# sundy-li/databend

Hardware: AMD Instinct MI355X
Metric: input rows/sec aggregated (filter + hash GROUP BY), % HBM roofline (higher is better)
Workload: dtype int16 key / u64 count; 1 GPU; clickbench_q8_adv_engine_id; rows_per_gpu=100000000, input_copies=4, groups=32, selected_rows=629660, parallelism=single

## Files before the change

databend_amd/csrc/abi_exp.hpp:

```cpp
#pragma once
#include "abi_internal.hpp"

static int exp_fused_fin(dbg_agg_handle* h, const FinState& F, FusedFin& ff) {
    const Spec& S = h->spec;
    {
        static const bool dense_on = X_ENV("DBG_X_DENSE") && X_ENV("DBG_X_DENSE")[0] == '1';
        const int kt = S.key_types[0].type;
        const u32 kw = (kt == DBG_INT8 || kt == DBG_UINT8) ? 1 : ((kt == DBG_INT16 || kt == DBG_UINT16) ? 2 : 0);
        const bool co = S.n_aggs == 1 && S.aggs[0].kind == DBG_AGG_COUNT && S.aggs[0].arg_type < 0 && S.aggs[0].w0 == 1;
        if (dense_on && kw && co && h->def_clean && S.n_keys == 1) {
            if (!h->dense) {
                RETURN_IF(h->dense.ensure(65536 + 1024));
                HIPCHECK(hipMemsetAsync(h->dense, 0, (65536 + 1024) * 8, h->stream));
            }
            ff.dense = h->dense;
            ff.dense_n = kw == 1 ? 256u : 65536u;
        }
    }
    static u64* x_trace = nullptr;
    static std::vector<u64> x_init;
    if (kPhaseTrace && X_ENV("DBG_X_TRACE")) {
        if (!x_trace) {
            RETURN_IF(dev_alloc((void**)&x_trace, 4096 * 128));
            x_init.assign(16, 0);
            x_init[0] = x_init[1] = ~0ULL;
            atexit([] {
                std::vector<u64> hb(4096 * 16);
                hipDeviceSynchronize();
                hipMemcpy(hb.data(), x_trace, hb.size() * 8, hipMemcpyDeviceToHost);
                std::vector<std::vector<double>> d(14);
                for (int k = 0; k < 4096; ++k) {
                    const u64* r = &hb[k * 16];
                    if (r[0] == 0 || r[0] == ~0ULL || r[6] == 0) continue;
                    for (int p = 1; p <= 14; ++p) d[p - 1].push_back((double)(r[p] - r[0]) * 0.01);
                }
                const char* nm[] = {"first WG stream end", "last WG stream end", "last block_flush end",
                                    "ticket (last WG)", "table copied", "finalize end", "fin: scanned",
                                    "fin: groups written", "fin: bits packed", "fin: counters read",
                                    "tail: view+counts", "tail: prefix", "tail: t0 loads", "tail: t0 merged"};
                for (int p = 0; p < 14; ++p) {
                    if (d[p].empty()) continue;
                    std::sort(d[p].begin(), d[p].end());
                    fprintf(stderr, "trace %-22s median %7.2f us  (n=%zu)\n", nm[p], d[p][d[p].size() / 2], d[p].size());
                }
            });
        }
        ff.trace = x_trace + (F.seq & 4095) * 16;
        HIPCHECK(hipMemcpyAsync(ff.trace, x_init.data(), 128, hipMemcpyHostToDevice, h->stream));
    }
    return DBG_OK;
}

static int exp_pp_trace(dbg_agg_handle* h, PPAggOut& o) {
    static u64* x_pptrace = nullptr;
    if (kPhaseTrace && X_ENV("DBG_X_PPTRACE")) {
        if (!x_pptrace) {
            RETURN_IF(dev_alloc((void**)&x_pptrace, 64));
            HIPCHECK(hipMemset(x_pptrace, 0, 64));
            atexit([] {
                u64 v[8];
                hipDeviceSynchronize();
                hipMemcpy(v, x_pptrace, 64, hipMemcpyDeviceToHost);
                const double n = v[5] ? (double)v[5] : 1.0;
                fprintf(stderr, "pptrace raw us/partition [0..4] %.2f %.2f %.2f %.2f %.2f (spec kernel: load+hash, stage, insert, "
                                "emit, barriers)\n", v[0] * 0.01 / n, v[1] * 0.01 / n, v[2] * 0.01 / n, v[3] * 0.01 / n, v[4] * 0.01 / n);
                fprintf(stderr, "pptrace partitions %llu groups/partition %.0f  per partition us: insert %.2f sync %.2f "
                                "atomic %.2f write %.2f tail %.2f\n", (unsigned long long)v[5], v[6] / n, v[0] * 0.01 / n,
                        v[1] * 0.01 / n, v[2] * 0.01 / n, v[3] * 0.01 / n, v[4] * 0.01 / n);
            });
        }
        o.trace = x_pptrace;
// ... 4 lines not shown
```

databend_amd/csrc/abi_finalize.hip:

```cpp
#include "abi_exp.hpp"

static void note_observed(dbg_agg_handle* h) {
    const u64 rows = h->table_rows > h->remerged ? h->table_rows - h->remerged : 0;
    if (h->pp || !rows) return;
    h->obs_rows = rows;
    h->obs_groups = h->n_groups;
}

static void publish_groups(const dbg_agg_handle* h, uint64_t* n_groups, uint64_t* string_bytes) {
    if (n_groups) *n_groups = h->n_groups;
    if (string_bytes)
        for (int c = 0; c < h->spec.n_keys; ++c) string_bytes[c] = h->string_bytes[c];
}

bool groups_known(dbg_agg_handle* h, u64 groups, const u64* str_tot, const FinState* caps, uint64_t* n_groups,
                  uint64_t* string_bytes) {
    const Spec& S = h->spec;
    h->n_groups = groups;
    note_observed(h);
    h->string_bytes.assign(S.n_keys, 0);
    bool short_buf = caps && groups > caps->max_groups;
    for (int c = 0; c < S.n_keys; ++c) {
        if (S.key_types[c].type != DBG_STRING) continue;
        h->string_bytes[c] = str_tot[c];
// ... 252 lines not shown
        if (e != hipSuccess) return fail(DBG_ERR_DEVICE, std::string("partitioned insert (direct stage): ") + hipGetErrorString(e));
        launch_finish_outputs(h->stream, od, totals, S.n_keys, S.n_aggs);
    } else if (fuse) {
        FusedFin ff;
        ff.out = od;
        ff.totals = totals;
        ff.host_mirror = h->hcounters_dev;
        ff.seq = F.seq;
        ff.recycle = h->recycle;
        ff.on = 1;
        ff.table_empty = h->def_clean ? 1 : 0;
        ff.chain_tagged = 0;
        ff.trace = nullptr;
        ff.dense = nullptr;
        ff.dense_n = 0;
        if ((F.seq / FIN_SEQ_TAG_PERIOD) != h->scr_period) {
            HIPCHECK(hipMemsetAsync(h->scratch, 0, scr_words(h->scr_blocks, (u32)S.stride_words) * 8, h->stream));
            h->scr_period = F.seq / FIN_SEQ_TAG_PERIOD;
        }
        RETURN_IF(exp_fused_fin(h, F, ff));
        h->def_on = false;
        prof::Scope ps("agg_insert", h->stream);
        note_insert(h, launch_insert(h->stream, h->dspec, S, h->dbatches, h->def_bid, h->def_rows, false, t, true, &h->def_hb, &ff));
    } else if (small) {
        prof::Scope ps("finalize_small", h->stream);
        launch_finalize_small(h->stream, h->dspec, h->dbatches, t, od, totals, F.zero_copy ? h->hcounters_dev : nullptr,
                              h->recycle && F.zero_copy, F.seq);
    } else {
        prof::Scope ps("write_results", h->stream);
        launch_write_results(h->stream, h->dspec, S, h->dbatches, t, h->d_pos, h->d_str_pos, od);
        launch_finish_outputs(h->stream, od, totals, S.n_keys, S.n_aggs);
    }
    if (!F.zero_copy) {
        HIPCHECK(hipMemcpyAsync(h->hcounters, h->counters, CNT_WORDS * 8, hipMemcpyDeviceToHost, h->stream));
        HIPCHECK(hipMemcpyAsync(h->hcounters + CNT_WORDS, totals, 8 * (S.n_keys + 1), hipMemcpyDeviceToHost, h->stream));
    }
    F.active = true;
    return DBG_OK;
}

static int fin_complete(dbg_agg_handle* h, bool* retry, uint64_t* n_groups, uint64_t* string_bytes) {
    FinState& F = h->fin;
    *retry = false;
    F.active = false;
    if (h->pp) return pp_fin_complete(h, n_groups, string_bytes);
    bool recycled = false;
// ... 3 lines not shown
    } else {
        volatile u64* hseq = h->hcounters + CNT_WORDS + 2 + DBG_MAX_KEYS;
        volatile u64* hcomp = h->hcounters + MIRROR_COMPACT;
        bool seen = false, compact = false;
        auto t0 = std::chrono::steady_clock::now();
        for (u64 it = 0;; ++it) {
            if (__atomic_load_n(hseq, __ATOMIC_ACQUIRE) == F.seq) {
                seen = true;
                break;
            }
            const u64 cw = __atomic_load_n(hcomp, __ATOMIC_ACQUIRE);
            if ((cw >> 25) == (F.seq & ((1ULL << 39) - 1))) {
                for (int w = 0; w < CNT_WORDS; ++w) h->hcounters[w] = 0;
                h->hcounters[CNT_CLAIMS] = cw & 0xFFFFFF;
                h->hcounters[CNT_WORDS] = cw & 0xFFFFFF;
                for (int c = 0; c < DBG_MAX_KEYS; ++c) h->hcounters[CNT_WORDS + 1 + c] = 0;
                h->hcounters[CNT_WORDS + 1 + DBG_MAX_KEYS] = (cw >> 24) & 1;
                seen = compact = true;
                break;
            }
            if ((it & 255) == 255 && std::chrono::steady_clock::now() - t0 > std::chrono::milliseconds(20)) break;
            __builtin_ia32_pause();
        }
        if (!seen) HIPCHECK(hipStreamSynchronize(h->stream));
        HIPCHECK(hipGetLastError());
        recycled = h->hcounters[CNT_WORDS + 1 + DBG_MAX_KEYS] != 0;
    }
    h->uploads_pending = false;
    if (F.direct) {
        F.direct = false;
        if (h->hcounters[CNT_WORDS] == ~0ULL) {
            h->def_part = true;
            RETURN_IF(part_flush(h));
            *retry = true;
            return DBG_OK;
        }
        h->hcounters[CNT_CLAIMS] = h->hcounters[CNT_WORDS];
        recycled = true;
    }
    RETURN_IF(err_bits_fail(h->hcounters[CNT_ERR], ERR_OVF_LOST | ERR_MINMAX_SPIN | ERR_CHAIN_SPIN | ERR_FIXED_INCOMPLETE));
    if (h->hcounters[CNT_OVF_ROWS] || h->hcounters[CNT_OVF_RECS]) {
        RETURN_IF(resolve_overflow(h));
        *retry = true;
        return DBG_OK;
    }
    h->pending_rows = h->pending_recs = 0;
    const u64* tot = h->hcounters + CNT_WORDS;
// ... 98 lines not shown
    for (int a = 0; a < h->spec.n_aggs; ++a)
        if (h->src_kinds[a] == DBG_AGG_AVG_SQL)
            return fail(DBG_ERR_UNSUPPORTED, "serialized states: SQL avg is sum and count in the reference plan");
    return result_impl(h, out_states, out_keys, on_device, true);
}

int dbg_agg_finalize_into(dbg_agg_handle* h, dbg_out_column* out_aggs, dbg_out_column* out_keys, uint64_t max_groups,
                          const uint64_t* max_string_bytes, uint64_t* n_groups, uint64_t* string_bytes) {
    RETURN_IF(dbg_agg_finalize_into_async(h, out_aggs, out_keys, max_groups, max_string_bytes));
    return dbg_agg_finalize_wait(h, n_groups, string_bytes);
}

int dbg_agg_finalize_into_async(dbg_agg_handle* h, dbg_out_column* out_aggs, dbg_out_column* out_keys, uint64_t max_groups,
                                const uint64_t* max_string_bytes) {
    if (!h || !out_aggs || !out_keys) return fail(DBG_ERR_INVALID, "null argument");
    if (has_str_minmax(h->spec))
        return fail(DBG_ERR_UNSUPPORTED, std::string("dbg_agg_finalize_into_async: ") + handle_local_reason(h->spec));
    if (h->fin.active) return fail(DBG_ERR_INVALID, "a finalize is already in flight: dbg_agg_finalize_wait first");
    HIPCHECK(hipSetDevice(h->device));
    RETURN_IF(fin_setup(h, out_aggs, out_keys, max_groups, max_string_bytes));
    return fin_launch(h);
}

int dbg_agg_finalize_wait(dbg_agg_handle* h, uint64_t* n_groups, uint64_t* string_bytes) {
    if (!h || !n_groups) return fail(DBG_ERR_INVALID, "null argument");
    if (!h->fin.active) return fail(DBG_ERR_INVALID, "no finalize in flight");
    HIPCHECK(hipSetDevice(h->device));
    RETURN_IF(flush_pending(h));
    for (int round = 0; round < 3; ++round) {
        if (round) RETURN_IF(fin_launch(h));
        bool retry = false;
        int rc = fin_complete(h, &retry, n_groups, string_bytes);
        if (rc != DBG_OK || !retry) return rc;
    }
    return fail(DBG_ERR_INTERNAL, "finalize did not converge");
}
}
```

databend_amd/csrc/agg.hip:

```cpp
#include <cstdlib>
#include <cstring>
#include <limits>
#include <type_traits>

#include "legacy.hpp"
#include "agg.hpp"
#include <hip/hip_ext.h>
#include "agg_dev.hpp"

#define BLOCK 256
#define SLOTS_PER_THREAD 8
#define SLOTS_PER_BLOCK (BLOCK * SLOTS_PER_THREAD)
#define LDS_BUDGET_BYTES (32 * 1024)
#define LDS_PROBE_CAP 64
#define FLUSH_ROUND 16



__device__ __forceinline__ u64 pack_key(const Spec& S, const DCol* keys, u64 i) {
    u64 k = 0;
    for (int c = 0; c < S.n_keys; ++c) {
        const DCol& col = keys[c];
        bool v = dcol_valid(col, i);
        if (col.nullable) k |= (u64)(v ? 1 : 0) << (8 * S.voff[c]);
// ... 2430 lines not shown
        default: return v >= k;
    }
}

template <typename T>
__device__ __forceinline__ T vget(const v4u& y, int j) {
    constexpr int W = sizeof(T);
    if constexpr (W == 8) {
        u32 lo = j ? y.z : y.x, hi = j ? y.w : y.y;
        return (T)(((u64)hi << 32) | lo);
    } else {
        int wi = (j * W) >> 2;
        u32 word = wi == 0 ? y.x : (wi == 1 ? y.y : (wi == 2 ? y.z : y.w));
        return (T)(word >> (((j * W) & 3) * 8));
    }
}

#define WQ 128
#define WQW 384

template <typename T, bool PRED, int NT, bool CO>
__global__ void __launch_bounds__(NT) agg_insert_fast_kernel(const Spec* __restrict__ spec, const BatchDesc* __restrict__ batches,
                                                               u32 bid, u64 rows, TableDesc t, u32 lds_slots,
                                                               T lo, T hi, int negate, FusedFin ff) {
    extern __shared__ __attribute__((aligned(16))) u64 lds[];
    constexpr int V = 16 / sizeof(T);
    const Spec& S = *spec;
    const BatchDesc& B = batches[bid];
    const T* __restrict__ col = (const T*)B.keys[0].data;
    const u32 sw = S.stride_words;
    u32* lcount = (u32*)(lds + (u64)lds_slots * sw);
    const u32 lmask = lds_slots - 1;
    const u32 llimit = lds_slots - lds_slots / 4;
    const int lane = threadIdx.x & 63, wave = threadIdx.x >> 6;
    u64* qkey = lds + (u64)lds_slots * sw + 2 + (u64)wave * WQW;
    u64* qrow = qkey + WQ;
    v4u* vq = (v4u*)qkey;
    u64* vqb = qkey + 2 * WQ;
    if (kPhaseTrace && ff.trace && threadIdx.x == 0) atomicMin((unsigned long long*)ff.trace, (unsigned long long)__builtin_amdgcn_s_memrealtime());
    lds_table_init<false>(S, lds, lds_slots, sw, NT);
    if (threadIdx.x < 4) lcount[threadIdx.x] = 0;
    __syncthreads();
    u32 my_claims = 0;
    u32 my_ovf = 0;

    auto pass = [&](T v) -> bool { return ((v >= lo) & (v <= hi)) ^ (negate != 0); };

    auto process = [&](u64 key, u64 i) {
        int ls = lds_find<true>(S, batches, nullptr, i, key, 0, lds, lmask, sw, lcount, llimit);
        if (ls >= 0) {
            wptr<AS_LDS> st = asp<AS_LDS>(lds + (u64)ls * sw);
            if (CO) at_add<AS_LDS>(st + 1, 1ULL);
            else apply_row<AS_LDS, false, false>(S, st, B, i, batches, bid);
            return;
        }
        bool claimed;
        u64 gs = g_find<true>(S, batches, nullptr, i, key, 0, t, t.probe_limit, claimed);
        if (gs == ~0ULL) {
            push_ovf_row(t, bid, i);
            my_ovf++;
            return;
        }
        my_claims += claimed ? 1 : 0;
        wptr<AS_GLB> gst = asp<AS_GLB>(t.slots + gs * t.stride_words);
        if (CO) at_add<AS_GLB>(gst + 1, 1ULL);
// ... 135 lines not shown
                    qkey[pos] = key_of(y[u], j);
                    qrow[pos] = base[u] + j;
                    pos++;
                }
            }
            qn += tot;
            while (qn >= 64) {
                __builtin_amdgcn_wave_barrier();
                drain64();
            }
        } else {
#pragma unroll
            for (int u = 0; u < FAST_UNROLL; ++u) {
                u32 mm = m[u];
                while (mm) {
                    int j = __builtin_ctz(mm);
                    mm &= mm - 1;
                    process(key_of(y[u], j), base[u] + j);
                }
            }
        }
    };

    const u64 nvec = rows / V;
    gv4p vp = (gv4p)col;
    const u64 gstride = (u64)gridDim.x * NT;
    u64 k = (u64)blockIdx.x * NT + threadIdx.x;
    const u64 step = (u64)FAST_UNROLL * gstride;
    const u64 lastv = nvec ? nvec - 1 : 0;
    constexpr u64 TAIL_CH = (u64)NT * FAST_UNROLL;
    const bool dyn = TAIL_ON && ff.on && t.scratch != nullptr && gridDim.x > 1 && gridDim.x <= t.scr_blocks;
    u64 nstat = nvec, nch = 0;
    if (dyn) {
        nstat = ((nvec * 4 / 5) / step) * step;
        nch = (nvec - nstat + TAIL_CH - 1) / TAIL_CH;
    }
    u64 tail_grab = 0;
    if (dyn && nch && threadIdx.x == 0) tail_grab = atomicAdd((unsigned long long*)(t.counters + CNT_TAIL), 1ULL);
    v4u y[FAST_UNROLL];
#pragma unroll
    for (int u = 0; u < FAST_UNROLL; ++u) {
        u64 idx = k + u * gstride;
        y[u] = __builtin_nontemporal_load(vp + (idx < nstat ? idx : lastv));
    }
    while (__ballot(k < nstat) != 0) {
        const u64 kn = k + step;
        v4u yn[FAST_UNROLL];
#pragma unroll
        for (int u = 0; u < FAST_UNROLL; ++u) {
            u64 idx = kn + u * gstride;
            yn[u] = __builtin_nontemporal_load(vp + (idx < nstat ? idx : lastv));
        }
        u64 bases[FAST_UNROLL];
        u32 actm = 0;
#pragma unroll
        for (int u = 0; u < FAST_UNROLL; ++u) {
            u64 idx = k + u * gstride;
            actm |= (idx < nstat ? 1u : 0u) << u;
            bases[u] = idx * V;
        }
        handle_group(y, bases, FAST_UNROLL, actm);
#pragma unroll
        for (int u = 0; u < FAST_UNROLL; ++u) y[u] = yn[u];
        k = kn;
    }
    if (dyn && nch) {
        __shared__ u32 tail_id[2];
// ... 67 lines not shown
    }
    if (ff.on && t.scratch != nullptr && gridDim.x > 1 && gridDim.x <= t.scr_blocks) {
        if constexpr (CO && sizeof(T) <= 2) {
            if (kChainTagged && ff.chain_tagged && lds_slots <= 4 * NT) {
                fused_chain_tagged<T>(S, batches, B, lds, lds_slots, sw, lcount, NT, t, my_claims, my_ovf, ff);
                return;
            }
        }
        fused_chain<T, CO>(S, batches, B, lds, lds_slots, sw, lcount, NT, t, my_claims, my_ovf, ff);
        return;
    }
    block_flush<true, false, false, false>(S, batches, B, lds, lds_slots, sw, lcount, NT, t, my_claims);
    if (kPhaseTrace && ff.trace && threadIdx.x == 0) atomicMax((unsigned long long*)ff.trace + 3, (unsigned long long)__builtin_amdgcn_s_memrealtime());
    if (ff.on) fused_finalize(S, batches, t, lds, ff);
}


bool prof_ext_events(hipEvent_t* a, hipEvent_t* b);

static size_t fast_shmem(size_t table_bytes) { return table_bytes + (size_t)(1024 / 64) * WQW * 8; }
static size_t fast_table_bytes(const Spec& S) { return (size_t)lds_slots_for(S, 16 * 1024) * S.stride_words * 8 + 16; }

template <typename T>
static void launch_fast_t(hipStream_t s, const Spec* dspec, const BatchDesc* batches, u32 bid, u64 rows, const TableDesc& t,
                          u32 lslots, size_t table_bytes, bool pred, int op, i64 c, int count_only, const FusedFin* fused) {
    constexpr u64 V = 16 / sizeof(T);
    typedef __int128 W;
    const W tmin = (W)std::numeric_limits<T>::min(), tmax = (W)std::numeric_limits<T>::max();
    const W C = std::is_signed<T>::value ? (W)c : (W)(u64)c;
    W lo = 1, hi = 0;
    int neg = 0;
    auto all = [&]() { lo = tmin; hi = tmax; };
    switch (op) {
        case DBG_CMP_EQ: if (C >= tmin && C <= tmax) lo = hi = C; break;
        case DBG_CMP_NE: neg = 1; if (C >= tmin && C <= tmax) lo = hi = C; break;
        case DBG_CMP_LT: if (C > tmax) all(); else if (C > tmin) { lo = tmin; hi = C - 1; } break;
        case DBG_CMP_LE: if (C >= tmax) all(); else if (C >= tmin) { lo = tmin; hi = C; } break;
        case DBG_CMP_GT: if (C < tmin) all(); else if (C < tmax) { lo = C + 1; hi = tmax; } break;
        default: if (C <= tmin) all(); else if (C <= tmax) { lo = C; hi = tmax; } break;
    }
    if (lo > hi) { lo = 1; hi = 0; }
    const int nt = 1024;
    static_assert(FIN_NT == 1024, "the fused finalize runs on the insert's workgroup");
    static const u64 x_grid = X_ENV("DBG_X_FAST_GRID") ? (u64)atoll(X_ENV("DBG_X_FAST_GRID")) : 0;
    const u64 max_blocks = (x_grid && fused && fused->dense) ? x_grid : 256;
    size_t shmem = fast_shmem(table_bytes);
    FusedFin ff;
    if (fused) ff = *fused;
    else memset(&ff, 0, sizeof(ff));
    u64 quantum = V * (u64)nt * FAST_UNROLL;
    u64 blocks = (rows + quantum - 1) / quantum;
    if (blocks > max_blocks) blocks = max_blocks;
    if (blocks > DBG_INSERT_MAX_BLOCKS) blocks = DBG_INSERT_MAX_BLOCKS;
    if (blocks < 1) blocks = 1;
    static_assert(FAST_UNROLL >= 1 && V * 1024 * FAST_UNROLL < (1ULL << CNT1_BITS), "one grid round of a workgroup fits a level-1 count");
    ff.chain_tagged = blocks <= CHAIN_TAGGED_MAX_BLOCKS && rows / blocks + V * (u64)nt + V < (1ULL << CNT1_BITS);
    hipEvent_t ev0 = nullptr, ev1 = nullptr;
    const bool ext = prof_ext_events(&ev0, &ev1);
#define FAST_LAUNCH(P, N, F)                                                                                                     \
    do {                                                                                                                         \
        if (ext)                                                                                                                 \
            hipExtLaunchKernelGGL((agg_insert_fast_kernel<T, P, N, F>), dim3((u32)blocks), dim3(N), shmem, s, ev0, ev1, 0, dspec, \
                                  batches, bid, rows, t, lslots, (T)lo, (T)hi, neg, ff);                                        \
        else                                                                                                                     \
            hipLaunchKernelGGL((agg_insert_fast_kernel<T, P, N, F>), dim3((u32)blocks), dim3(N), shmem, s, dspec, batches, bid, \
                               rows, t, lslots, (T)lo, (T)hi, neg, ff);                                                          \
    } while (0)
    if (count_only) {
        if (pred) FAST_LAUNCH(true, 1024, true); else FAST_LAUNCH(false, 1024, true);
    } else {
        if (pred) FAST_LAUNCH(true, 1024, false); else FAST_LAUNCH(false, 1024, false);
    }
#undef FAST_LAUNCH
}

static bool fast_eligible(const Spec& S, const BatchDesc& hb, bool records) {
    if (records || !S.inline_keys || S.n_keys != 1 || S.key_types[0].nullable) return false;
    for (int a = 0; a < S.n_aggs; ++a)
        if ((S.aggs[a].kind == DBG_AGG_MIN || S.aggs[a].kind == DBG_AGG_MAX) && S.aggs[a].mmk == MMK_STR) return false;
    for (int a = 0; a < S.n_aggs; ++a)
        if (S.aggs[a].arg_type == DBG_DECIMAL256) return false;
    const DCol& k = hb.keys[0];
    int ty = k.type;
    bool intlike = (ty >= DBG_INT8 && ty <= DBG_UINT64) || ty == DBG_DATE || ty == DBG_TIMESTAMP;
    if (!intlike || k.layout != LAYOUT_ARROW || ((uintptr_t)k.data & 15)) return false;
    if (hb.n_nodes == 0) return true;
    if (hb.n_nodes != 1) return false;
    const DNode& n = hb.nodes[0];
    const DCol& f = hb.fcols[n.col];
    return n.op == DBG_PRED_CMP_CONST && f.data == k.data && f.type == ty && !f.nullable;
}

bool insert_can_fuse(const Spec& S, const BatchDesc& hb, u64 cap) {
    return hb.rows > 0 && fast_eligible(S, hb, false) && cap + 1 <= FUSED_FIN_SLOTS &&
           (cap + 1) * S.stride_words * 8 <= fast_shmem(fast_table_bytes(S));
}

InsertPath launch_insert(hipStream_t s, const Spec* dspec, const Spec& S, const BatchDesc* batches, u32 bid, u64 rows, bool records,
                         const TableDesc& t, bool use_lds, const BatchDesc* hb, const FusedFin* fused) {
    if (rows == 0) return INS_NONE;
    if (hb && use_lds && fast_eligible(S, *hb, records)) {
        u32 lslots = lds_slots_for(S, 16 * 1024);
        size_t shmem = fast_table_bytes(S);
        bool pred = hb->n_nodes == 1;
        int op = pred ? hb->nodes[0].cmp : 0;
        i64 c = pred ? hb->nodes[0].i64v : 0;
        int count_only = S.n_aggs == 1 && S.aggs[0].kind == DBG_AGG_COUNT && S.aggs[0].arg_type < 0 && S.aggs[0].w0 == 1;
        const InsertPath path = pred ? INS_FAST_PRED : INS_FAST;
        switch (hb->keys[0].type) {
            case DBG_INT8: launch_fast_t<int8_t>(s, dspec, batches, bid, rows, t, lslots, shmem, pred, op, c, count_only, fused); return path;
            case DBG_UINT8: launch_fast_t<uint8_t>(s, dspec, batches, bid, rows, t, lslots, shmem, pred, op, c, count_only, fused); return path;
            case DBG_INT16: launch_fast_t<int16_t>(s, dspec, batches, bid, rows, t, lslots, shmem, pred, op, c, count_only, fused); return path;
            case DBG_UINT16: launch_fast_t<uint16_t>(s, dspec, batches, bid, rows, t, lslots, shmem, pred, op, c, count_only, fused); return path;
            case DBG_INT32: case DBG_DATE: launch_fast_t<int32_t>(s, dspec, batches, bid, rows, t, lslots, shmem, pred, op, c, count_only, fused); return path;
            case DBG_UINT32: launch_fast_t<uint32_t>(s, dspec, batches, bid, rows, t, lslots, shmem, pred, op, c, count_only, fused); return path;
            case DBG_INT64: case DBG_TIMESTAMP: launch_fast_t<int64_t>(s, dspec, batches, bid, rows, t, lslots, shmem, pred, op, c, count_only, fused); return path;
            case DBG_UINT64: launch_fast_t<uint64_t>(s, dspec, batches, bid, rows, t, lslots, shmem, pred, op, c, count_only, fused); return path;
        }
    }
    if (!records && use_lds && hb && S.kc_word && t.cap + 1 > SHORT_MAX_SLOTS && str1_eligible(S, *hb, rows)) {
        const u32 lsw = (u32)S.kc_word + 1 + KC_KEY_WORDS;
        static const u32 x_mode = X_ENV("DBG_X_STR1") ? (u32)atoi(X_ENV("DBG_X_STR1")) : 0;
        static const u32 x_lds = X_ENV("DBG_X_STR1_LDS") ? (u32)atoi(X_ENV("DBG_X_STR1_LDS")) * 1024 : STR1_LDS_BUDGET;
        static const u32 fper = X_ENV("DBG_X_STR1_FLUSH") ? (u32)atoi(X_ENV("DBG_X_STR1_FLUSH")) : 4;
        u32 ls = 1;
        while ((ls * 2) * lsw * 8 <= x_lds) ls *= 2;
        const size_t shmem = (size_t)ls * lsw * 8 + 32 + (size_t)STR1_QCAP * 8;
        u64 blocks = (rows + (u64)STR1_NT * 16 - 1) / ((u64)STR1_NT * 16);
        if (blocks > DBG_INSERT_MAX_BLOCKS) blocks = DBG_INSERT_MAX_BLOCKS;
        if (blocks < 1) blocks = 1;
        u64 rpb = ((rows + blocks - 1) / blocks + 1) & ~1ULL;
        blocks = (rows + rpb - 1) / rpb;
        if (hb->n_nodes) hipLaunchKernelGGL(agg_insert_str1_kernel<true>, dim3((u32)blocks), dim3(STR1_NT), shmem, s, dspec, batches, bid, rows, rpb, t, ls, fper, x_mode);
        else hipLaunchKernelGGL(agg_insert_str1_kernel<false>, dim3((u32)blocks), dim3(STR1_NT), shmem, s, dspec, batches, bid, rows, rpb, t, ls, fper, x_mode);
        return hb->n_nodes ? INS_STR1_PRED : INS_STR1;
    }
    u32 lslots = use_lds ? lds_slots_for(S, LDS_BUDGET_BYTES) : 1;
    static const int x_short = X_ENV("DBG_X_SHORT") ? atoi(X_ENV("DBG_X_SHORT")) : 1;
    static const u32 x_rep = X_ENV("DBG_X_SHORT_REP") ? (u32)atoi(X_ENV("DBG_X_SHORT_REP")) : 0;
    const bool x_noshort = x_short == 0;
// ... 402 lines not shown
```

databend_amd/ffi.py:

```python
from __future__ import annotations

import ctypes as C
import os

from . import abi

_HERE = os.path.dirname(os.path.abspath(__file__))
LIB_PATH = os.environ.get("DBGPU_LIB") or os.path.join(_HERE, "libdbgpu_agg.so")
_LIB = None

EXPORTED = [
    "dbg_version", "dbg_last_error", "dbg_device_count", "dbg_agg_result_type", "dbg_agg_create",
    "dbg_agg_destroy", "dbg_agg_set_stream", "dbg_agg_reset", "dbg_agg_add_groups", "dbg_agg_finalize",
    "dbg_agg_result", "dbg_agg_finalize_into", "dbg_agg_set_recycle", "dbg_agg_set_partition_keys", "dbg_agg_finalize_into_async", "dbg_agg_finalize_wait", "dbg_agg_record_width", "dbg_agg_partition", "dbg_agg_export_records",
    "dbg_agg_merge_records", "dbg_agg_export_fixed", "dbg_agg_capacity", "dbg_agg_merge_fixed", "dbg_filter_select", "dbg_take_fixed", "dbg_sort_limit_indices", "dbg_sort_limit_multi", "dbg_agg_compact", "dbg_agg_retained_bytes", "dbg_prof_enable", "dbg_prof_reset",
    "dbg_prof_get", "dbg_prof_marker", "dbg_datagen", "dbg_agg_set_strategy", "dbg_agg_get_strategy", "dbg_agg_get_pp_stats", "dbg_agg_insert_paths",
    "dbg_agg_record_layout", "dbg_agg_set_host_staging", "dbg_agg_result_string_bytes",
    "dbg_take_string", "dbg_legacy_hash_method", "dbg_legacy_group_hash", "dbg_agg_serialized_stride", "dbg_agg_result_serialized", "dbg_agg_merge_serialized", "dbg_comm_get_unique_id", "dbg_comm_create", "dbg_comm_destroy", "dbg_agg_exchange",
    "dbg_agg_payload_counts", "dbg_agg_payload_export", "dbg_agg_payload_import", "dbg_agg_exchange_payload",
    "dbg_payload_exchange_plan", "dbg_merge_exchange_plan", "dbg_agg_payload_counts_from", "dbg_agg_payload_export_from",
    "dbg_agg_payload_import_chunks", "dbg_agg_exchange_payload_chunk",
    "dbg_scan_create", "dbg_scan_destroy", "dbg_parquet_chunk_rows", "dbg_parquet_decode",
    "dbg_native_decode", "dbg_like_pattern_kind", "dbg_like_match_host", "dbg_like_kernel_counts", "dbg_like_force_kernel",
]


class DbgError(RuntimeError):

    def __init__(self, code: int, msg: str):
        super().__init__(f"[{code}] {msg}")
        self.code = code


class DecimalOverflow(DbgError):
    pass


# ... 22 lines not shown
        L.dbg_agg_destroy.restype = None
        L.dbg_agg_set_stream.argtypes = [VP, VP]
        L.dbg_agg_reset.argtypes = [VP]
        L.dbg_agg_add_groups.argtypes = [VP, P(abi.dbg_column), P(abi.dbg_column), P(abi.dbg_filter), U64, C.c_int]
        L.dbg_agg_finalize.argtypes = [VP, P(U64), P(U64)]
        L.dbg_agg_result.argtypes = [VP, P(abi.dbg_out_column), P(abi.dbg_out_column), C.c_int]
        L.dbg_agg_result_string_bytes.argtypes = [VP, P(U64)]
        L.dbg_agg_finalize_into.argtypes = [VP, P(abi.dbg_out_column), P(abi.dbg_out_column), U64, P(U64), P(U64), P(U64)]
        L.dbg_agg_set_recycle.argtypes = [VP, C.c_int]
        L.dbg_agg_set_partition_keys.argtypes = [VP, C.c_int]
        L.dbg_agg_set_host_staging.argtypes = [VP, U64]
        L.dbg_comm_get_unique_id.argtypes = [VP]
        L.dbg_comm_create.argtypes = [VP, C.c_int, C.c_int, C.c_int, P(VP)]
        L.dbg_comm_destroy.argtypes = [VP]
        L.dbg_comm_destroy.restype = None
        L.dbg_agg_exchange.argtypes = [VP, VP, VP, P(abi.dbg_exchange_stats)]
        L.dbg_agg_set_strategy.argtypes = [VP, C.c_int]
        L.dbg_agg_record_layout.argtypes = [P(abi.dbg_agg_params), P(abi.dbg_record_layout)]
        L.dbg_agg_get_strategy.argtypes = [VP, P(C.c_int), P(U64)]
        L.dbg_agg_get_pp_stats.argtypes = [VP, P(C.c_uint32), P(U64)]
        L.dbg_agg_insert_paths.argtypes = [VP, P(U64), I32]
        L.dbg_agg_finalize_into_async.argtypes = [VP, P(abi.dbg_out_column), P(abi.dbg_out_column), U64, P(U64)]
        L.dbg_agg_finalize_wait.argtypes = [VP, P(U64), P(U64)]
        L.dbg_agg_record_width.argtypes = [VP, P(C.c_uint32)]
        L.dbg_agg_partition.argtypes = [VP, C.c_uint32, C.c_int, P(U64), P(U64)]
        L.dbg_agg_export_records.argtypes = [VP, VP, VP]
        L.dbg_agg_merge_records.argtypes = [VP, VP, VP, I32, P(U64), P(U64)]
        L.dbg_agg_export_fixed.argtypes = [VP, VP, U64]
        L.dbg_agg_capacity.argtypes = [VP, P(U64)]
        L.dbg_agg_merge_fixed.argtypes = [VP, VP, I32, U64]
        L.dbg_filter_select.argtypes = [P(abi.dbg_filter), U64, VP, P(U64), VP]
        L.dbg_take_fixed.argtypes = [P(abi.dbg_column), VP, U64, VP, VP, VP]
        L.dbg_agg_serialized_stride.argtypes = [VP, P(C.c_uint32)]
        L.dbg_agg_result_serialized.argtypes = [VP, P(abi.dbg_out_column), P(abi.dbg_out_column), C.c_int]
        L.dbg_agg_merge_serialized.argtypes = [VP, P(abi.dbg_column), P(abi.dbg_column), U64, C.c_int]
        L.dbg_legacy_hash_method.argtypes = [P(abi.dbg_datatype), C.c_int, P(C.c_int), P(C.c_uint32)]
        L.dbg_legacy_group_hash.argtypes = [P(abi.dbg_column), C.c_int, U64, VP, VP, C.c_int, VP]
        L.dbg_take_string.argtypes = [P(abi.dbg_column), VP, U64, VP, VP, U64, VP, P(U64), VP]
        L.dbg_sort_limit_indices.argtypes = [P(abi.dbg_column), U64, C.c_int, C.c_int, U64, VP, P(U64), VP]
        L.dbg_agg_compact.argtypes = [VP, P(C.c_int)]
        L.dbg_agg_retained_bytes.argtypes = [VP, P(U64)]
        L.dbg_sort_limit_multi.argtypes = [P(abi.dbg_column), C.c_int, P(C.c_int), P(C.c_int), U64, U64, VP, P(U64), VP]
        L.dbg_prof_enable.argtypes = [C.c_int]
        L.dbg_prof_get.argtypes = [C.c_int, P(C.c_char_p), P(C.c_double), P(U64)]
        L.dbg_prof_marker.argtypes = [VP]
        L.dbg_agg_payload_counts.argtypes = [VP, P(U64), P(C.c_uint32)]
# ... 57 lines not shown
```

databend_amd/workloads.py:

```python
from __future__ import annotations

import ctypes as C
import math
import time
from dataclasses import dataclass
from typing import Dict, List, Optional

import numpy as np

from . import abi
from . import column as col
from .aggregates import AggregateFunctionFactory
from .aggregator import AggregateHashTable, AggregatorParams, HashTableConfig
from .column import Column, DataType
from .device import DeviceColumn, empty
from .ffi import check, lib
from .filter import FilterProgram, cmp

BASE_SEED = 0xDA7ABE7D
F = AggregateFunctionFactory.instance()


def _torch():
    import torch
# ... 224 lines not shown
            break
        return self._publish(o, n.value, list(sb))

    def finalize_async(self, h, parity=0):
        o = self._outset(parity)
        check(lib().dbg_agg_finalize_into_async(h, o.oa, o.ok, o.cap, o.scap))

    def finalize_wait(self, h, parity=0):
        n = C.c_uint64()
        sb = (C.c_uint64 * len(self.shape.keys))()
        o = self._outset(parity)
        rc = lib().dbg_agg_finalize_wait(h, C.byref(n), sb)
        if rc == abi.DBG_ERR_INVALID and (n.value > o.cap or any(x > y for x, y in zip(sb, o.scap))):
            self._alloc_out(int(n.value * 1.25) + 1, [int(x * 1.25) + 1 for x in sb], parity)
            return self.finalize_into(h, parity)
        check(rc)
        return self._publish(o, n.value, list(sb))

    def enable_pipeline(self, mode: str = ""):
        import os
        torch = _torch()
        if getattr(self, "tables", None):
            return
        self.pipe_mode = mode or os.environ.get("DBG_PIPE_MODE", "single")
        t1 = AggregateHashTable(self.params, HashTableConfig(True, self._capacity_hint))
        check(lib().dbg_agg_set_recycle(t1.h, 1))
        self.tables = [self.table, t1]
        sa = torch.cuda.Stream()
        self.streams = [sa, sa if self.pipe_mode == "single" else torch.cuda.Stream()]
        for t, st in zip(self.tables, self.streams):
            t.set_stream(st)
        self._inflight = None

    def pipe_step(self, k: int):
        p = k % 2
        t = self.tables[p]
        self.insert(k, t)
        self.finalize_async(t.h, p)
        n = self.pipe_drain()
        self._inflight = (t.h, p)
        return n

    def pipe_drain(self):
        f, self._inflight = getattr(self, "_inflight", None), None
        return self.finalize_wait(*f) if f else 0

    def results_host(self):
        keys = [c.to_host_n(self.n_groups) if hasattr(c, "to_host_n") else _dev_to_host(c, self.n_groups) for c in self.out_keys]
        aggs = [_dev_to_host(c, self.n_groups) for c in self.out_aggs]
        return keys, aggs

    def close(self):
        for t in getattr(self, "tables", None) or [self.table]:
            t.close()


class _OutSet:

    def __init__(self, runner, cap, scap):
        self.aggs = [empty(t, cap) for t in runner.result_types]
        self.keys = [empty(t, cap, string_bytes=scap[j]) for j, t in enumerate(runner.params.group_data_types)]
# ... 47 lines not shown
```

include/dbgpu_agg.h:

```cpp
#ifndef DBGPU_AGG_H
#define DBGPU_AGG_H

#include <stdint.h>

#ifdef __cplusplus
extern "C" {
#endif

#define DBG_ABI_VERSION 1

enum {
    DBG_OK = 0,
    DBG_ERR_OVERFLOW = 1,
    DBG_ERR_OOM = 2,
    DBG_ERR_UNSUPPORTED = 3,
    DBG_ERR_INTERNAL = 4,
    DBG_ERR_INVALID = 5,
    DBG_ERR_DEVICE = 6
};

typedef enum {
    DBG_INT8 = 0,
    DBG_INT16 = 1,
    DBG_INT32 = 2,
// ... 122 lines not shown
int dbg_agg_set_stream(dbg_agg_handle* h, void* hip_stream);
int dbg_agg_reset(dbg_agg_handle* h);

int dbg_agg_add_groups(dbg_agg_handle* h, const dbg_column* group_cols, const dbg_column* arg_cols,
                       const dbg_filter* filter, uint64_t rows, int on_device);

int dbg_agg_finalize(dbg_agg_handle* h, uint64_t* n_groups, uint64_t* string_bytes);

int dbg_agg_result(dbg_agg_handle* h, dbg_out_column* out_aggs, dbg_out_column* out_keys, int on_device);
int dbg_agg_result_string_bytes(dbg_agg_handle* h, uint64_t* agg_string_bytes );
int dbg_agg_serialized_stride(dbg_agg_handle* h, uint32_t* stride );
int dbg_agg_result_serialized(dbg_agg_handle* h, dbg_out_column* out_states, dbg_out_column* out_keys, int on_device);

int dbg_agg_merge_serialized(dbg_agg_handle* h, const dbg_column* state_cols, const dbg_column* group_cols, uint64_t rows,
                             int on_device);

int dbg_agg_finalize_into(dbg_agg_handle* h, dbg_out_column* out_aggs, dbg_out_column* out_keys,
                          uint64_t max_groups, const uint64_t* max_string_bytes, uint64_t* n_groups,
                          uint64_t* string_bytes);

int dbg_agg_finalize_into_async(dbg_agg_handle* h, dbg_out_column* out_aggs, dbg_out_column* out_keys,
                                uint64_t max_groups, const uint64_t* max_string_bytes);
int dbg_agg_finalize_wait(dbg_agg_handle* h, uint64_t* n_groups, uint64_t* string_bytes);

int dbg_agg_set_recycle(dbg_agg_handle* h, int on);
int dbg_agg_set_partition_keys(dbg_agg_handle* h, int n_keys);

int dbg_agg_set_host_staging(dbg_agg_handle* h, uint64_t rows);

enum { DBG_STRATEGY_AUTO = 0, DBG_STRATEGY_TABLE = 1, DBG_STRATEGY_PARTITIONED = 2 };
int dbg_agg_set_strategy(dbg_agg_handle* h, int strategy);
int dbg_agg_get_strategy(dbg_agg_handle* h, int* partitioned, uint64_t* extra_rounds);
int dbg_agg_get_pp_stats(dbg_agg_handle* h, uint32_t* final_bits, uint64_t* spilled_partitions);
enum {
    DBG_INSERT_GENERIC = 0,
    DBG_INSERT_GENERIC_LENPRED = 1,
    DBG_INSERT_FAST = 2,
    DBG_INSERT_FAST_PRED = 3,
    DBG_INSERT_STR1 = 4,
    DBG_INSERT_STR1_PRED = 5,
    DBG_INSERT_SHORT = 6,
    DBG_INSERT_PP_GENERIC = 7,
    DBG_INSERT_PP_FIXED = 8,
    DBG_INSERT_PP_STR = 9,
    DBG_INSERT_N_PATHS = 10
};
// ... 94 lines not shown
```

Baseline: 2533 billion rows/s.

## Add single-call step API, dual-stream pipeline default, and early key-column prefetch

Adds dbg_agg_step_async, which does reset, add_groups, finalize setup and launch in one FFI call, and routes the Python pipeline through it to cut per-step host overhead. The default pipeline mode changes from a single shared stream to 'dual', which uses the default (None) streams. The fast insert kernel now takes the key pointer and stride as kernel arguments instead of loading them from device descriptors, and issues the first unrolled nontemporal loads before the LDS table init, replacing __syncthreads with a raw waitcnt plus barrier. Trace instrumentation is also restructured to measure the host gap between launches; the stream-mode change alters ordering semantics and may add overlap or contention.

```diff
diff --git a/databend_amd/csrc/abi_exp.hpp b/databend_amd/csrc/abi_exp.hpp
--- a/databend_amd/csrc/abi_exp.hpp
+++ b/databend_amd/csrc/abi_exp.hpp
@@ -1,5 +1,74 @@
 #pragma once
 #include "abi_internal.hpp"
+
+struct XTrace {
+    u64* ring = nullptr;
+    u64 launches = 0;
+    std::vector<u64> init;
+    std::chrono::steady_clock::time_point seen_at;
+    bool seen = false;
+    std::vector<double> host_us;
+};
+inline XTrace& x_tr() {
+    static XTrace x;
+    return x;
+}
+inline bool x_trace_on() {
+    static const bool on = kPhaseTrace && X_ENV("DBG_X_TRACE");
+    return on;
+}
+inline void exp_completion_seen() {
+    if (!x_trace_on()) return;
+    x_tr().seen_at = std::chrono::steady_clock::now();
+    x_tr().seen = true;
+}
+inline void exp_launch_returned() {
+    XTrace& X = x_tr();
+    if (!x_trace_on() || !X.seen) return;
+    X.host_us.push_back(std::chrono::duration<double, std::micro>(std::chrono::steady_clock::now() - X.seen_at).count());
+    X.seen = false;
+}
+inline void x_trace_dump() {
+    XTrace& X = x_tr();
+    std::vector<u64> hb(4096 * 16);
+    hipDeviceSynchronize();
+    hipMemcpy(hb.data(), X.ring, hb.size() * 8, hipMemcpyDeviceToHost);
+    auto median_line = [](const char* what, std::vector<double>& v) {
+        if (v.empty()) return;
+        std::sort(v.begin(), v.end());
+        fprintf(stderr, "trace %-44s median %7.2f us  min %7.2f  max %7.2f  (n=%zu)\n", what, v[v.size() / 2], v.front(), v.back(),
+                v.size());
+    };
+    auto whole = [](const u64* r) { return r[0] != 0 && r[0] != ~0ULL && r[1] != ~0ULL && r[6] != 0; };
+    std::vector<std::vector<double>> d(14);
+    for (int k = 0; k < 4096; ++k) {
+        const u64* r = &hb[k * 16];
+        if (!whole(r)) continue;
+        for (int p = 1; p <= 14; ++p)
+            if (r[p]) d[p - 1].push_back((double)(r[p] - r[0]) * 0.01);
+    }
+    const char* nm[] = {"first WG stream end", "last WG stream end", "last block_flush end",
+                        "ticket (last WG)", "table copied", "finalize end", "fin: scanned",
+                        "fin: groups written", "fin: bits packed", "fin: counters read",
+                        "tail: view+counts", "tail: prefix", "tail: t0 loads", "tail: t0 merged"};
+    for (int p = 0; p < 14; ++p) {
+        if (d[p].empty()) continue;
+        std::sort(d[p].begin(), d[p].end());
+        fprintf(stderr, "trace %-22s median %7.2f us  (n=%zu)\n", nm[p], d[p][d[p].size() / 2], d[p].size());
+    }
+    std::vector<double> vs_stream, vs_fin;
+    const u64 n = X.launches, first = n > 4096 ? n - 4096 : 0;
+    for (u64 j = first; j + 1 < n; ++j) {
+        const u64* a = &hb[(j & 4095) * 16];
+        const u64* b = &hb[((j + 1) & 4095) * 16];
+        if (!whole(a) || !whole(b)) continue;
+        vs_stream.push_back((double)(int64_t)(b[0] - a[1]) * 0.01);
+        vs_fin.push_back((double)(int64_t)(b[0] - a[6]) * 0.01);
+    }
+    median_line("next first WG start - first WG stream end", vs_stream);
+    median_line("next first WG start - finalize end", vs_fin);
+    median_line("host: completion seen -> next launch returned", X.host_us);
+}
 
 static int exp_fused_fin(dbg_agg_handle* h, const FinState& F, FusedFin& ff) {
     const Spec& S = h->spec;
@@ -17,36 +86,16 @@
             ff.dense_n = kw == 1 ? 256u : 65536u;
         }
     }
-    static u64* x_trace = nullptr;
-    static std::vector<u64> x_init;
-    if (kPhaseTrace && X_ENV("DBG_X_TRACE")) {
-        if (!x_trace) {
-            RETURN_IF(dev_alloc((void**)&x_trace, 4096 * 128));
-            x_init.assign(16, 0);
-            x_init[0] = x_init[1] = ~0ULL;
-            atexit([] {
-                std::vector<u64> hb(4096 * 16);
-                hipDeviceSynchronize();
-                hipMemcpy(hb.data(), x_trace, hb.size() * 8, hipMemcpyDeviceToHost);
-                std::vector<std::vector<double>> d(14);
-                for (int k = 0; k < 4096; ++k) {
-                    const u64* r = &hb[k * 16];
-                    if (r[0] == 0 || r[0] == ~0ULL || r[6] == 0) continue;
-                    for (int p = 1; p <= 14; ++p) d[p - 1].push_back((double)(r[p] - r[0]) * 0.01);
-                }
-                const char* nm[] = {"first WG stream end", "last WG stream end", "last block_flush end",
-                                    "ticket (last WG)", "table copied", "finalize end", "fin: scanned",
-                                    "fin: groups written", "fin: bits packed", "fin: counters read",
-                                    "tail: view+counts", "tail: prefix", "tail: t0 loads", "tail: t0 merged"};
-                for (int p = 0; p < 14; ++p) {
-                    if (d[p].empty()) continue;
-                    std::sort(d[p].begin(), d[p].end());
-                    fprintf(stderr, "trace %-22s median %7.2f us  (n=%zu)\n", nm[p], d[p][d[p].size() / 2], d[p].size());
-                }
-            });
+    if (x_trace_on()) {
+        XTrace& X = x_tr();
+        if (!X.ring) {
+            RETURN_IF(dev_alloc((void**)&X.ring, 4096 * 128));
+            X.init.assign(16, 0);
+            X.init[0] = X.init[1] = ~0ULL;
+            atexit(x_trace_dump);
         }
-        ff.trace = x_trace + (F.seq & 4095) * 16;
-        HIPCHECK(hipMemcpyAsync(ff.trace, x_init.data(), 128, hipMemcpyHostToDevice, h->stream));
+        ff.trace = X.ring + (X.launches++ & 4095) * 16;
+        HIPCHECK(hipMemcpyAsync(ff.trace, X.init.data(), 128, hipMemcpyHostToDevice, h->stream));
     }
     return DBG_OK;
 }
diff --git a/databend_amd/csrc/abi_finalize.hip b/databend_amd/csrc/abi_finalize.hip
--- a/databend_amd/csrc/abi_finalize.hip
+++ b/databend_amd/csrc/abi_finalize.hip
@@ -298,6 +298,7 @@
         h->def_on = false;
         prof::Scope ps("agg_insert", h->stream);
         note_insert(h, launch_insert(h->stream, h->dspec, S, h->dbatches, h->def_bid, h->def_rows, false, t, true, &h->def_hb, &ff));
+        exp_launch_returned();
     } else if (small) {
         prof::Scope ps("finalize_small", h->stream);
         launch_finalize_small(h->stream, h->dspec, h->dbatches, t, od, totals, F.zero_copy ? h->hcounters_dev : nullptr,
@@ -347,7 +348,8 @@
             if ((it & 255) == 255 && std::chrono::steady_clock::now() - t0 > std::chrono::milliseconds(20)) break;
             __builtin_ia32_pause();
         }
-        if (!seen) HIPCHECK(hipStreamSynchronize(h->stream));
+        if (seen) exp_completion_seen();
+        else HIPCHECK(hipStreamSynchronize(h->stream));
         HIPCHECK(hipGetLastError());
         recycled = h->hcounters[CNT_WORDS + 1 + DBG_MAX_KEYS] != 0;
     }
@@ -492,6 +494,19 @@
     return fin_launch(h);
 }
 
+int dbg_agg_step_async(dbg_agg_handle* h, const dbg_column* group_cols, const dbg_column* arg_cols, const dbg_filter* filter,
+                       uint64_t rows, dbg_out_column* out_aggs, dbg_out_column* out_keys, uint64_t max_groups,
+                       const uint64_t* max_string_bytes) {
+    if (!h || !group_cols || !out_aggs || !out_keys) return fail(DBG_ERR_INVALID, "null argument");
+    if (has_str_minmax(h->spec))
+        return fail(DBG_ERR_UNSUPPORTED, std::string("dbg_agg_step_async: ") + handle_local_reason(h->spec));
+    if (h->fin.active) return fail(DBG_ERR_INVALID, "a finalize is already in flight: dbg_agg_finalize_wait first");
+    RETURN_IF(dbg_agg_reset(h));
+    RETURN_IF(dbg_agg_add_groups(h, group_cols, arg_cols, filter, rows, 1));
+    RETURN_IF(fin_setup(h, out_aggs, out_keys, max_groups, max_string_bytes));
+    return fin_launch(h);
+}
+
 int dbg_agg_finalize_wait(dbg_agg_handle* h, uint64_t* n_groups, uint64_t* string_bytes) {
     if (!h || !n_groups) return fail(DBG_ERR_INVALID, "null argument");
     if (!h->fin.active) return fail(DBG_ERR_INVALID, "no finalize in flight");
diff --git a/databend_amd/csrc/agg.hip b/databend_amd/csrc/agg.hip
--- a/databend_amd/csrc/agg.hip
+++ b/databend_amd/csrc/agg.hip
@@ -2476,13 +2476,14 @@
 template <typename T, bool PRED, int NT, bool CO>
 __global__ void __launch_bounds__(NT) agg_insert_fast_kernel(const Spec* __restrict__ spec, const BatchDesc* __restrict__ batches,
                                                                u32 bid, u64 rows, TableDesc t, u32 lds_slots,
-                                                               T lo, T hi, int negate, FusedFin ff) {
+                                                               T lo, T hi, int negate, FusedFin ff, const void* key0,
+                                                               u32 stride_words) {
     extern __shared__ __attribute__((aligned(16))) u64 lds[];
     constexpr int V = 16 / sizeof(T);
     const Spec& S = *spec;
     const BatchDesc& B = batches[bid];
-    const T* __restrict__ col = (const T*)B.keys[0].data;
-    const u32 sw = S.stride_words;
+    const T* __restrict__ col = (const T*)key0;
+    const u32 sw = stride_words;
     u32* lcount = (u32*)(lds + (u64)lds_slots * sw);
     const u32 lmask = lds_slots - 1;
     const u32 llimit = lds_slots - lds_slots / 4;
@@ -2492,9 +2493,28 @@
     v4u* vq = (v4u*)qkey;
     u64* vqb = qkey + 2 * WQ;
     if (kPhaseTrace && ff.trace && threadIdx.x == 0) atomicMin((unsigned long long*)ff.trace, (unsigned long long)__builtin_amdgcn_s_memrealtime());
+    const u64 nvec = rows / V;
+    gv4p vp = (gv4p)col;
+    const u64 gstride = (u64)gridDim.x * NT;
+    u64 k = (u64)blockIdx.x * NT + threadIdx.x;
+    const u64 step = (u64)FAST_UNROLL * gstride;
+    const u64 lastv = nvec ? nvec - 1 : 0;
+    constexpr u64 TAIL_CH = (u64)NT * FAST_UNROLL;
+    const bool dyn = TAIL_ON && ff.on && t.scratch != nullptr && gridDim.x > 1 && gridDim.x <= t.scr_blocks;
+    u64 nstat = nvec, nch = 0;
+    if (dyn) {
+        nstat = ((nvec * 4 / 5) / step) * step;
+        nch = (nvec - nstat + TAIL_CH - 1) / TAIL_CH;
+    }
+    v4u y[FAST_UNROLL];
+#pragma unroll
+    for (int u = 0; u < FAST_UNROLL; ++u) {
+        u64 idx = k + u * gstride;
+        y[u] = __builtin_nontemporal_load(vp + (idx < nstat ? idx : lastv));
+    }
     lds_table_init<false>(S, lds, lds_slots, sw, NT);
     if (threadIdx.x < 4) lcount[threadIdx.x] = 0;
-    __syncthreads();
+    asm volatile("s_waitcnt lgkmcnt(0)\n\ts_barrier" ::: "memory");
     u32 my_claims = 0;
     u32 my_ovf = 0;
 
@@ -2676,27 +2696,8 @@
         }
     };
 
-    const u64 nvec = rows / V;
-    gv4p vp = (gv4p)col;
-    const u64 gstride = (u64)gridDim.x * NT;
-    u64 k = (u64)blockIdx.x * NT + threadIdx.x;
-    const u64 step = (u64)FAST_UNROLL * gstride;
-    const u64 lastv = nvec ? nvec - 1 : 0;
-    constexpr u64 TAIL_CH = (u64)NT * FAST_UNROLL;
-    const bool dyn = TAIL_ON && ff.on && t.scratch != nullptr && gridDim.x > 1 && gridDim.x <= t.scr_blocks;
-    u64 nstat = nvec, nch = 0;
-    if (dyn) {
-        nstat = ((nvec * 4 / 5) / step) * step;
-        nch = (nvec - nstat + TAIL_CH - 1) / TAIL_CH;
-    }
     u64 tail_grab = 0;
     if (dyn && nch && threadIdx.x == 0) tail_grab = atomicAdd((unsigned long long*)(t.counters + CNT_TAIL), 1ULL);
-    v4u y[FAST_UNROLL];
-#pragma unroll
-    for (int u = 0; u < FAST_UNROLL; ++u) {
-        u64 idx = k + u * gstride;
-        y[u] = __builtin_nontemporal_load(vp + (idx < nstat ? idx : lastv));
-    }
     while (__ballot(k < nstat) != 0) {
         const u64 kn = k + step;
         v4u yn[FAST_UNROLL];
@@ -2810,8 +2811,9 @@
 static size_t fast_table_bytes(const Spec& S) { return (size_t)lds_slots_for(S, 16 * 1024) * S.stride_words * 8 + 16; }
 
 template <typename T>
-static void launch_fast_t(hipStream_t s, const Spec* dspec, const BatchDesc* batches, u32 bid, u64 rows, const TableDesc& t,
-                          u32 lslots, size_t table_bytes, bool pred, int op, i64 c, int count_only, const FusedFin* fused) {
+static void launch_fast_t(hipStream_t s, const Spec* dspec, const Spec& S, const void* key0, const BatchDesc* batches, u32 bid, u64 rows,
+                          const TableDesc& t, u32 lslots, size_t table_bytes, bool pred, int op, i64 c, int count_only,
+                          const FusedFin* fused) {
     constexpr u64 V = 16 / sizeof(T);
     typedef __int128 W;
     const W tmin = (W)std::numeric_limits<T>::min(), tmax = (W)std::numeric_limits<T>::max();
@@ -2849,10 +2851,10 @@
     do {                                                                                                                         \
         if (ext)                                                                                                                 \
             hipExtLaunchKernelGGL((agg_insert_fast_kernel<T, P, N, F>), dim3((u32)blocks), dim3(N), shmem, s, ev0, ev1, 0, dspec, \
-                                  batches, bid, rows, t, lslots, (T)lo, (T)hi, neg, ff);                                        \
+                                  batches, bid, rows, t, lslots, (T)lo, (T)hi, neg, ff, key0, (u32)S.stride_words);             \
         else                                                                                                                     \
             hipLaunchKernelGGL((agg_insert_fast_kernel<T, P, N, F>), dim3((u32)blocks), dim3(N), shmem, s, dspec, batches, bid, \
-                               rows, t, lslots, (T)lo, (T)hi, neg, ff);                                                          \
+                               rows, t, lslots, (T)lo, (T)hi, neg, ff, key0, (u32)S.stride_words);                               \
     } while (0)
     if (count_only) {
         if (pred) FAST_LAUNCH(true, 1024, true); else FAST_LAUNCH(false, 1024, true);
@@ -2896,14 +2898,14 @@
         int count_only = S.n_aggs == 1 && S.aggs[0].kind == DBG_AGG_COUNT && S.aggs[0].arg_type < 0 && S.aggs[0].w0 == 1;
         const InsertPath path = pred ? INS_FAST_PRED : INS_FAST;
         switch (hb->keys[0].type) {
-            case DBG_INT8: launch_fast_t<int8_t>(s, dspec, batches, bid, rows, t, lslots, shmem, pred, op, c, count_only, fused); return path;
-            case DBG_UINT8: launch_fast_t<uint8_t>(s, dspec, batches, bid, rows, t, lslots, shmem, pred, op, c, count_only, fused); return path;
-            case DBG_INT16: launch_fast_t<int16_t>(s, dspec, batches, bid, rows, t, lslots, shmem, pred, op, c, count_only, fused); return path;
-            case DBG_UINT16: launch_fast_t<uint16_t>(s, dspec, batches, bid, rows, t, lslots, shmem, pred, op, c, count_only, fused); return path;
-            case DBG_INT32: case DBG_DATE: launch_fast_t<int32_t>(s, dspec, batches, bid, rows, t, lslots, shmem, pred, op, c, count_only, fused); return path;
-            case DBG_UINT32: launch_fast_t<uint32_t>(s, dspec, batches, bid, rows, t, lslots, shmem, pred, op, c, count_only, fused); return path;
-            case DBG_INT64: case DBG_TIMESTAMP: launch_fast_t<int64_t>(s, dspec, batches, bid, rows, t, lslots, shmem, pred, op, c, count_only, fused); return path;
-            case DBG_UINT64: launch_fast_t<uint64_t>(s, dspec, batches, bid, rows, t, lslots, shmem, pred, op, c, count_only, fused); return path;
+            case DBG_INT8: launch_fast_t<int8_t>(s, dspec, S, hb->keys[0].data, batches, bid, rows, t, lslots, shmem, pred, op, c, count_only, fused); return path;
+            case DBG_UINT8: launch_fast_t<uint8_t>(s, dspec, S, hb->keys[0].data, batches, bid, rows, t, lslots, shmem, pred, op, c, count_only, fused); return path;
+            case DBG_INT16: launch_fast_t<int16_t>(s, dspec, S, hb->keys[0].data, batches, bid, rows, t, lslots, shmem, pred, op, c, count_only, fused); return path;
+            case DBG_UINT16: launch_fast_t<uint16_t>(s, dspec, S, hb->keys[0].data, batches, bid, rows, t, lslots, shmem, pred, op, c, count_only, fused); return path;
+            case DBG_INT32: case DBG_DATE: launch_fast_t<int32_t>(s, dspec, S, hb->keys[0].data, batches, bid, rows, t, lslots, shmem, pred, op, c, count_only, fused); return path;
+            case DBG_UINT32: launch_fast_t<uint32_t>(s, dspec, S, hb->keys[0].data, batches, bid, rows, t, lslots, shmem, pred, op, c, count_only, fused); return path;
+            case DBG_INT64: case DBG_TIMESTAMP: launch_fast_t<int64_t>(s, dspec, S, hb->keys[0].data, batches, bid, rows, t, lslots, shmem, pred, op, c, count_only, fused); return path;
+            case DBG_UINT64: launch_fast_t<uint64_t>(s, dspec, S, hb->keys[0].data, batches, bid, rows, t, lslots, shmem, pred, op, c, count_only, fused); return path;
         }
     }
     if (!records && use_lds && hb && S.kc_word && t.cap + 1 > SHORT_MAX_SLOTS && str1_eligible(S, *hb, rows)) {
diff --git a/databend_amd/ffi.py b/databend_amd/ffi.py
--- a/databend_amd/ffi.py
+++ b/databend_amd/ffi.py
@@ -12,7 +12,7 @@
 EXPORTED = [
     "dbg_version", "dbg_last_error", "dbg_device_count", "dbg_agg_result_type", "dbg_agg_create",
     "dbg_agg_destroy", "dbg_agg_set_stream", "dbg_agg_reset", "dbg_agg_add_groups", "dbg_agg_finalize",
-    "dbg_agg_result", "dbg_agg_finalize_into", "dbg_agg_set_recycle", "dbg_agg_set_partition_keys", "dbg_agg_finalize_into_async", "dbg_agg_finalize_wait", "dbg_agg_record_width", "dbg_agg_partition", "dbg_agg_export_records",
+    "dbg_agg_result", "dbg_agg_finalize_into", "dbg_agg_set_recycle", "dbg_agg_set_partition_keys", "dbg_agg_finalize_into_async", "dbg_agg_finalize_wait", "dbg_agg_step_async", "dbg_agg_record_width", "dbg_agg_partition", "dbg_agg_export_records",
     "dbg_agg_merge_records", "dbg_agg_export_fixed", "dbg_agg_capacity", "dbg_agg_merge_fixed", "dbg_filter_select", "dbg_take_fixed", "dbg_sort_limit_indices", "dbg_sort_limit_multi", "dbg_agg_compact", "dbg_agg_retained_bytes", "dbg_prof_enable", "dbg_prof_reset",
     "dbg_prof_get", "dbg_prof_marker", "dbg_datagen", "dbg_agg_set_strategy", "dbg_agg_get_strategy", "dbg_agg_get_pp_stats", "dbg_agg_insert_paths",
     "dbg_agg_record_layout", "dbg_agg_set_host_staging", "dbg_agg_result_string_bytes",
@@ -81,6 +81,8 @@
         L.dbg_agg_insert_paths.argtypes = [VP, P(U64), I32]
         L.dbg_agg_finalize_into_async.argtypes = [VP, P(abi.dbg_out_column), P(abi.dbg_out_column), U64, P(U64)]
         L.dbg_agg_finalize_wait.argtypes = [VP, P(U64), P(U64)]
+        L.dbg_agg_step_async.argtypes = [VP, P(abi.dbg_column), P(abi.dbg_column), P(abi.dbg_filter), U64, P(abi.dbg_out_column),
+                                         P(abi.dbg_out_column), U64, P(U64)]
         L.dbg_agg_record_width.argtypes = [VP, P(C.c_uint32)]
         L.dbg_agg_partition.argtypes = [VP, C.c_uint32, C.c_int, P(U64), P(U64)]
         L.dbg_agg_export_records.argtypes = [VP, VP, VP]
diff --git a/databend_amd/workloads.py b/databend_amd/workloads.py
--- a/databend_amd/workloads.py
+++ b/databend_amd/workloads.py
@@ -270,12 +270,17 @@
         torch = _torch()
         if getattr(self, "tables", None):
             return
-        self.pipe_mode = mode or os.environ.get("DBG_PIPE_MODE", "single")
+        self.pipe_mode = mode or os.environ.get("DBG_PIPE_MODE", "dual")
+        if self.pipe_mode not in ("dual", "single", "pool"):
+            raise ValueError(f"pipeline mode {self.pipe_mode!r}: dual, single or pool")
         t1 = AggregateHashTable(self.params, HashTableConfig(True, self._capacity_hint))
         check(lib().dbg_agg_set_recycle(t1.h, 1))
         self.tables = [self.table, t1]
-        sa = torch.cuda.Stream()
-        self.streams = [sa, sa if self.pipe_mode == "single" else torch.cuda.Stream()]
+        if self.pipe_mode == "dual":
+            self.streams = [None, None]
+        else:
+            sa = torch.cuda.Stream()
+            self.streams = [sa, sa if self.pipe_mode == "single" else torch.cuda.Stream()]
         for t, st in zip(self.tables, self.streams):
             t.set_stream(st)
         self._inflight = None
@@ -283,8 +288,9 @@
     def pipe_step(self, k: int):
         p = k % 2
         t = self.tables[p]
-        self.insert(k, t)
-        self.finalize_async(t.h, p)
+        keys, args, fp = self._prepared(k % len(self.inputs))
+        o = self._outset(p)
+        check(lib().dbg_agg_step_async(t.h, keys, args, fp, self.rows, o.oa, o.ok, o.cap, o.scap))
         n = self.pipe_drain()
         self._inflight = (t.h, p)
         return n
diff --git a/include/dbgpu_agg.h b/include/dbgpu_agg.h
--- a/include/dbgpu_agg.h
+++ b/include/dbgpu_agg.h
@@ -168,6 +168,10 @@
 int dbg_agg_finalize_into_async(dbg_agg_handle* h, dbg_out_column* out_aggs, dbg_out_column* out_keys,
                                 uint64_t max_groups, const uint64_t* max_string_bytes);
 int dbg_agg_finalize_wait(dbg_agg_handle* h, uint64_t* n_groups, uint64_t* string_bytes);
+
+int dbg_agg_step_async(dbg_agg_handle* h, const dbg_column* group_cols, const dbg_column* arg_cols,
+                       const dbg_filter* filter, uint64_t rows, dbg_out_column* out_aggs, dbg_out_column* out_keys,
+                       uint64_t max_groups, const uint64_t* max_string_bytes);
 
 int dbg_agg_set_recycle(dbg_agg_handle* h, int on);
 int dbg_agg_set_partition_keys(dbg_agg_handle* h, int n_keys);
```

New measurement: 2912 billion rows/s (median of 6 runs). 1.15x the previous value.
